# omnirevolve/omnirevolve-image-processor

Hardware: AMD Instinct MI355X
Metric: Mpx/s end-to-end (color->order) (higher is better)
Workload: dtype u8/i32 raster + f32/f64 geometry; 1 GPU; 4096x4096 BGR image, 8 colour layers, stages 02->12 (k-means fit, masks, edges, contours, scale, sort, intra dedup, cross dedup, plot order), default A4 canvas 8400x11880; parallelism=one GPU, one pipeline per colour layer, ops_last_step_rank0=4261, exchange=none

## Files before the change

### omnirevolve-image-processor_amd/csrc/vec_common.h

```cpp
#pragma once
#include "orip_ctx.h"
#include "vec_serial.h"
#include "vsrc.h"
#include <algorithm>
#include <chrono>
#include <string>

template <class T> int vscan_excl(orip_ctx* c, const T* in, T* out, size_t n);
template <class K, class V> int vsort_pairs(orip_ctx* c, const K* kin, K* kout, const V* vin, V* vout, size_t n, int begin_bit, int end_bit, bool desc = false);
template <class T>
static inline int vread(orip_ctx* c, T* host, const T* dev, size_t n = 1) {
    HIPC(c, hipMemcpyAsync(host, dev, n * sizeof(T), hipMemcpyDeviceToHost, LN(c).stream));
    HIPC(c, hipStreamSynchronize(LN(c).stream));
    return 0;
}
struct PhaseTimer {
    orip_ctx* c; const bool on; std::string log; std::chrono::steady_clock::time_point prev;
    PhaseTimer(orip_ctx* ctx, const char* env) : c(ctx), on(getenv(env) != nullptr), prev(std::chrono::steady_clock::now()) {}
    double lap() {
        if (on) hipStreamSynchronize(LN(c).stream);
        const auto t = std::chrono::steady_clock::now(); const double ms = std::chrono::duration<double, std::milli>(t - prev).count(); prev = t;
        return ms;
    }
    void tick(const char* name) { if (on) { char b[64]; snprintf(b, sizeof b, " %s %.2f", name, lap()); log += b; } }
};

struct PolyFeat {
    int32_t x0, y0, x1, y1;
    int32_t sx, sy, ex, ey;
    int64_t n;
    float per;
    double arc;
    uint8_t closed;
};

#define ORIP_LONG_POLY 192
#define ORIP_LONG_CUM 128
static_assert(ORIP_LONG_POLY >= ORIP_LONG_CUM, "every polyline whose perimeter is summed from stored segment lengths must have had them stored");
static inline ESrc esrc_of(const DPolys& P) { return ESrc{P.off.as<int64_t>(), reinterpret_cast<const int2*>(P.pts.p)}; }
int vsrc_of(orip_ctx* c, const DPolys& P, VSrc& out);
#define ORIP_WITH_SRC(c, P, SRC, BODY)                                                         \
    do {                                                                                       \
        if (is_coded(P)) { VSrc SRC; ORIP_TRY(vsrc_of(c, P, SRC)); BODY }                      \
        else { const ESrc SRC = esrc_of(P); BODY }                                             \
    } while (0)
__device__ __forceinline__ int64_t last_le(const int64_t* off, int64_t n, int64_t v) {
    int64_t lo = 0, hi = n - 1;
    while (lo < hi) { const int64_t mid = (lo + hi + 1) >> 1; if (off[mid] <= v) lo = mid; else hi = mid - 1; }
    return lo;
}
__device__ __forceinline__ int64_t ub_u32(const unsigned* a, int64_t n, unsigned v) {
    int64_t lo = 0, hi = n;
    while (lo < hi) { int64_t mid = (lo + hi) >> 1; if (a[mid] <= v) lo = mid + 1; else hi = mid; }
    return lo;
}
template <class Cur> struct CurPt {
    Cur& c;
    __device__ __forceinline__ vs::IPt operator()(int64_t i) const { const int2 p = c.at(i); return vs::IPt{p.x, p.y}; }
};
enum : int {
    VF_PER = 1,
    VF_PER_HYPOT = 2,
    VF_ARC_CLOSED = 4,
    VF_ARC_OPEN = 8,
    VF_OPEN_VIEW = 16,
    VF_PER_REV = 32,
    VF_LEAVES_DONE = 64,
};
int vfeatures(orip_ctx* c, const DPolys& P, int what, PolyFeat* feat);
void vfeatures_short(orip_ctx* c, const VSrc& src, int64_t n, int what, PolyFeat* feat, float* per_rev);
int vlen_order(orip_ctx* c, const int64_t* off, int64_t n, unsigned* kin, unsigned* kout, unsigned* vin, unsigned* order);
int vfeatures_long_seg(orip_ctx* c, const VSrc& src, int64_t n, int64_t total, PolyFeat* feat, const unsigned* order, float* per_rev, const float* seg);
void vwalk_arcs(orip_ctx* c, const VSrc& src, int64_t n, PolyFeat* feat);

struct GatherDesc { int64_t begin; int64_t len; int32_t rev; int32_t src; };
int vgather(orip_ctx* c, const GatherDesc* d, int64_t n, const int32_t* src, DPolys& dst, int64_t known_total = -1);
int vgather_views(orip_ctx* c, const GatherDesc* d, int64_t n, const DPolys& src, DPolys& dst, int64_t known_total = -1);
int vgather_list(orip_ctx* c, const GatherDesc* d, int64_t n, const DPolys& src, DPolys& dst, int64_t known_total = -1);

#define ORIP_RUN_TILE 4096u
struct SlotPtsI2 { const int2* p; __device__ __forceinline__ int2 at(unsigned s) const { return p[s]; } };
struct SlotPtsF64 {
    const double* x; const double* y;
    __device__ __forceinline__ int2 at(unsigned s) const { return make_int2((int)x[s], (int)y[s]); }
};
template <class Pts> int orip_runs_to_polys(orip_ctx* c, Pts pts, const uint8_t* sflag, unsigned n_slots, DPolys& dst);

int vreorder(orip_ctx* c, DPolys& src, DPolys& dst, int kind, const orip_params08* prefetch08 = nullptr);
```

### omnirevolve-image-processor_amd/csrc/vector08a.hip

```cpp
#include "vec08.h"
#include <rocprim/rocprim.hpp>
#include <type_traits>
#include <vector>

namespace {

template <class Src>
__global__ __launch_bounds__(128) void k_split_small08(Src src, int64_t n_polys, orip_params08 P, const PolyFeat* __restrict__ feat,
                                                        unsigned* __restrict__ is_tap, unsigned* __restrict__ is_keep, int2* __restrict__ tap_xy, GatherDesc* __restrict__ kd) {
    int64_t i = (int64_t)blockIdx.x * blockDim.x + threadIdx.x;
    if (i > n_polys) return;
    if (i == n_polys) { is_tap[i] = 0; is_keep[i] = 0; return; }
    const int64_t n = src.len(i);
    unsigned tap = 0, keep = 0;
    GatherDesc g; g.begin = src.off[i]; g.len = n; g.rev = 0; g.src = (int32_t)i;
    if (n >= 2) {
        const int32_t x0 = feat[i].x0, x1 = feat[i].x1, y0 = feat[i].y0, y1 = feat[i].y1;
        double d = (double)max(x1 - x0, y1 - y0);
        if (d <= P.tap_diam && d <= P.tap_max_dim && n <= (int64_t)P.tap_max_v) {
            double per; float cx, cy, r;
            if constexpr (std::is_same<Src, ESrc>::value) {
                const int32_t* p = reinterpret_cast<const int32_t*>(src.pts + src.off[i]);
                per = (double)vs::pairwise_seglen_sum<0>(p, n);
                if (per <= P.tap_max_per) vs::min_enclosing_circle(p, n, cx, cy, r);
            } else {
                auto cu = src.cur(i);
                LocalPts<decltype(cu), 64> lp; lp.load(cu, (int)n);
                per = (double)vs::pairwise_seglen_sum<0>(lp.xy, n);
                if (per <= P.tap_max_per) vs::min_enclosing_circle(lp.xy, n, cx, cy, r);
            }
            if (per <= P.tap_max_per) { tap = 1; tap_xy[i] = make_int2((int)vs::round_half_even((double)cx), (int)vs::round_half_even((double)cy)); }
        }
        if (!tap && !(d < P.min_keep)) {
            keep = 1;
            if (feat[i].closed) g.len = n - 1;
        }
    }
    is_tap[i] = tap; is_keep[i] = keep; kd[i] = g;
}
template <class T>
__global__ __launch_bounds__(256) void k_compact(const unsigned* __restrict__ flag, const unsigned* __restrict__ scan, int64_t n, const T* __restrict__ in, T* __restrict__ out) {
    int64_t i = (int64_t)blockIdx.x * 256 + threadIdx.x;
    if (i < n && flag[i]) out[scan[i]] = in[i];
}

struct RsInfo { int64_t n_eff; double total; unsigned m; unsigned pass; };
__device__ __forceinline__ void rs_finish(RsInfo& r, float acc, int64_t n, double step) {
    r.total = (double)acc;
    if (r.total <= step) { r.pass = 1; r.m = (unsigned)n; }
    else r.m = (unsigned)ceil(r.total / step);
    if (r.m < 2) r.m = 0;
}
template <class Src>
__global__ __launch_bounds__(128) void k_cumlen(Src src, int64_t n_polys, double step, float* __restrict__ cum, RsInfo* __restrict__ info) {
    int64_t i = (int64_t)blockIdx.x * blockDim.x + threadIdx.x;
    if (i >= n_polys) return;
    auto cu = src.cur(i); int64_t n = src.len(i);
    float* s = cum + src.off[i];
    RsInfo r; r.n_eff = n; r.total = 0; r.m = 0; r.pass = 0;
    const int2 pf = cu.at(0);
    auto same_as_first = [&](int64_t k) { const int2 q = cu.at(k); return q.x == pf.x && q.y == pf.y; };
    if (n >= 2 && same_as_first(n - 1)) n -= 1;
    r.n_eff = n;
    if (n >= 2) {
        if (n > 2 && same_as_first(n - 1)) n -= 1;
        r.n_eff = n;
        if (n <= ORIP_LONG_CUM) {
            const CurPt<decltype(cu)> pt{cu};
            float acc = 0.f; s[0] = 0.f;
            for (int64_t k = 0; k + 1 < n; k++) { float sl = vs::seg_len_f32_p(pt, k); acc = (k == 0) ? sl : acc + sl; s[k + 1] = acc; }
            rs_finish(r, acc, n, step);
        }
    }
    info[i] = r;
}

__device__ __forceinline__ unsigned wave_incl_scan_u32(unsigned v) {
#define ORIP_DPP_ADD(ctrl, rowmask) v += (unsigned)__builtin_amdgcn_update_dpp(0, (int)v, ctrl, rowmask, 0xf, false);
    ORIP_DPP_ADD(0x111, 0xf) ORIP_DPP_ADD(0x112, 0xf) ORIP_DPP_ADD(0x114, 0xf) ORIP_DPP_ADD(0x118, 0xf)
    ORIP_DPP_ADD(0x142, 0xa) ORIP_DPP_ADD(0x143, 0xc)
#undef ORIP_DPP_ADD
    return v;
}
__device__ __forceinline__ unsigned wave_incl_scan_max_u32(unsigned v) {
#define ORIP_DPP_MAX(ctrl, rowmask) { const unsigned t_ = (unsigned)__builtin_amdgcn_update_dpp(0, (int)v, ctrl, rowmask, 0xf, false); v = t_ > v ? t_ : v; }
    ORIP_DPP_MAX(0x111, 0xf) ORIP_DPP_MAX(0x112, 0xf) ORIP_DPP_MAX(0x114, 0xf) ORIP_DPP_MAX(0x118, 0xf)
    ORIP_DPP_MAX(0x142, 0xa) ORIP_DPP_MAX(0x143, 0xc)
#undef ORIP_DPP_MAX
    return v;
}
__device__ __forceinline__ float cum_window(float dval, int lane, unsigned& E, unsigned& M) {
    const unsigned b = __float_as_uint(dval);
    const unsigned Ed = b >> 23, Md = Ed ? ((b & 0x7fffffu) | 0x800000u) : 0u;
    unsigned out = 0u; int first = 0;
    for (;;) {
        const int sh = (int)E - (int)Ed;
        const unsigned sc = (unsigned)(sh < 0 ? 0 : (sh > 31 ? 31 : sh));
        const unsigned rem = Md & ((1u << sc) - 1u), half = (1u << sc) >> 1;
        const bool live = lane >= first;
        const bool ev = live && (sh < 0 || (sc > 0u && rem == half));
        const unsigned r = (live && sh >= 0) ? (Md >> sc) + ((sc > 0u && rem > half) ? 1u : 0u) : 0u;
        const unsigned S = wave_incl_scan_u32(r);
        const unsigned long long em = __ballot(ev || (live && M + S >= 0x1000000u));
        const int f = em ? __builtin_ctzll(em) : 64;
        if (live && lane < f) out = (E << 23) | ((M + S) & 0x7fffffu);
        if (f == 64) { M += (unsigned)__builtin_amdgcn_readlane((int)S, 63); break; }
        const unsigned Mp = M + (f > first ? (unsigned)__builtin_amdgcn_readlane((int)S, f - 1) : 0u);
        const float pprev = __uint_as_float((E << 23) | (Mp & 0x7fffffu));
        const float pnew = __fadd_rn(pprev, __uint_as_float((unsigned)__builtin_amdgcn_readlane((int)b, f)));
        const unsigned nb = __float_as_uint(pnew);
        if (lane == f) out = nb;
        E = nb >> 23; M = E ? ((nb & 0x7fffffu) | 0x800000u) : 0u;
        first = f + 1;
        if (first == 64) break;
    }
    return __uint_as_float(out);
}
__device__ __forceinline__ float cum_state_value(unsigned E, unsigned M) { return __uint_as_float((E << 23) | (M & 0x7fffffu)); }
template <class Src>
__global__ __launch_bounds__(128) void k_cumlen2(Src src, const PolyFeat* __restrict__ feat07, int64_t n_polys, double step, float* __restrict__ cum, int64_t rev_off, RsInfo* __restrict__ info) {
    const int64_t gi = (int64_t)blockIdx.x * blockDim.x + threadIdx.x;
    if (gi >= 2 * n_polys) return;
    const int64_t i = gi < n_polys ? gi : gi - n_polys; const int dir0 = gi < n_polys ? 0 : 1;
    auto cu = src.cur(i); const int64_t nfull = src.len(i);
    const bool closed = feat07[i].closed != 0;
    for (int dir = dir0; dir <= dir0; dir++) {
        int64_t n = (dir == 0 && closed && nfull > 0) ? nfull - 1 : nfull;
        float* s = cum + (dir ? rev_off : 0) + src.off[i];
        auto P = [&](int64_t k) { return dir ? cu.at(nfull - 1 - k) : cu.at(k); };
        RsInfo r; r.n_eff = n; r.total = 0; r.m = 0; r.pass = 0;
        if (dir == 1 && closed) { r.n_eff = 0; info[n_polys + i] = r; continue; }
        const int2 pf = P(0);
        auto same_as_first = [&](int64_t k) { const int2 q = P(k); return q.x == pf.x && q.y == pf.y; };
        if (n >= 2 && same_as_first(n - 1)) n -= 1;
        r.n_eff = n;
        if (n >= 2) {
            if (n > 2 && same_as_first(n - 1)) n -= 1;
            r.n_eff = n;
            if (n <= ORIP_LONG_CUM) {
                float acc = 0.f; s[0] = 0.f;
                int2 a = P(0);
                for (int64_t k = 0; k + 1 < n; k++) {
                    const int2 b = P(k + 1);
                    float dx = (float)b.x - (float)a.x, dy = (float)b.y - (float)a.y; float qx = dx * dx, qy = dy * dy; const float sl = sqrtf(qx + qy);
                    acc = (k == 0) ? sl : acc + sl; s[k + 1] = acc; a = b;
                }
                rs_finish(r, acc, n, step);
            }
        }
        info[dir ? n_polys + i : i] = r;
    }
}
__device__ __forceinline__ int2 lane_succ(const int2 v, const int2 last, int lane) {
    int2 r;
    r.x = __builtin_amdgcn_update_dpp(0, v.x, 0x130 , 0xf, 0xf, true);
    r.y = __builtin_amdgcn_update_dpp(0, v.y, 0x130, 0xf, 0xf, true);
    if (lane == 63) r = last;
    return r;
}
template <class Src>
__device__ __forceinline__ void cumlen_long_wave(const Src& src, int64_t n_polys, double step, float* __restrict__ cum, int64_t rev_off, RsInfo* __restrict__ info,
                                                 const unsigned* __restrict__ ord, const bool rev, const float* __restrict__ seg, int64_t slot, int64_t n_slots, const int lane) {
    for (int64_t rr = slot; rr < n_polys; rr += n_slots) {
        const int64_t i = ord[rr];
        RsInfo r = info[rev ? n_polys + i : i];
        if (r.n_eff <= ORIP_LONG_CUM) continue;
        auto cu = src.cur(i); const int64_t nfull = src.len(i);
        float* s = cum + (rev ? rev_off : 0) + src.off[i];
        const int64_t ns = r.n_eff - 1;
        const float* sg = seg ? seg + src.off[i] : nullptr;
        const bool from_seg = sg != nullptr;
        float acc = 0.f; unsigned cE = 0u, cM = 0u;
        if (lane == 0) s[0] = 0.f;
        auto P = [&](int64_t k) { return cu.at(rev ? nfull - 1 - k : k); };
        auto request = [&](int64_t base, int2 (&p)[5], float (&fl)[4]) {
            if (from_seg) {
#pragma unroll
                for (int w = 0; w < 4; w++) { const int64_t k = base + 64 * w + lane; fl[w] = k < ns ? sg[rev ? nfull - 2 - k : k] : 0.f; }
            } else {
#pragma unroll
                for (int w = 0; w < 4; w++) { const int64_t k = base + 64 * w + lane; p[w] = k <= ns ? P(k) : make_int2(0, 0); }
                p[4] = base + 256 <= ns ? P(base + 256) : make_int2(0, 0);
            }
        };
        auto lengths = [&](int64_t base, const int2 (&p)[5], const float (&fl)[4], float (&sl)[4]) {
            if (from_seg) {
#pragma unroll
                for (int w = 0; w < 4; w++) sl[w] = fl[w];
                return;
            }
#pragma unroll
            for (int w = 0; w < 4; w++) {
                const int64_t k = base + 64 * w + lane;
                const int2 nx0 = w < 3 ? make_int2(__builtin_amdgcn_readlane(p[w + 1].x, 0), __builtin_amdgcn_readlane(p[w + 1].y, 0)) : p[4];
                const int2 b2 = lane_succ(p[w], nx0, lane);
                float dx = (float)b2.x - (float)p[w].x, dy = (float)b2.y - (float)p[w].y; float qx = dx * dx, qy = dy * dy;
                const float L = sqrtf(qx + qy);
                sl[w] = k < ns ? L : 0.f;
            }
        };
        int2 rp[5]; float rf[4] = {0.f, 0.f, 0.f, 0.f}; float cur[4];
        request(0, rp, rf); lengths(0, rp, rf, cur);
        for (int64_t base = 0; base < ns; base += 256) {
            request(base + 256, rp, rf);
#pragma unroll
            for (int w = 0; w < 4; w++) {
                const int64_t k = base + 64 * w + lane;
                const float pv = cum_window(cur[w], lane, cE, cM); acc = cum_state_value(cE, cM);
                if (k < ns) s[k + 1] = pv;
            }
            lengths(base + 256, rp, rf, cur);
        }
        if (lane == 0) { rs_finish(r, acc, r.n_eff, step); info[rev ? n_polys + i : i] = r; }
    }
}
template <class Src>
__global__ __launch_bounds__(64) void k_cumlen_long2(Src src, int64_t n_polys, double step, float* __restrict__ cum, int64_t rev_off, RsInfo* __restrict__ info, const unsigned* __restrict__ ord,
                                                     int dir0, const float* __restrict__ seg) {
    cumlen_long_wave<Src>(src, n_polys, step, cum, rev_off, info, ord, ((blockIdx.y + (unsigned)dir0) & 1u) != 0, seg, blockIdx.x, gridDim.x, threadIdx.x);
}
template <class Src>
__global__ __launch_bounds__(256) void k_seglen(Src src, int64_t n_polys, int64_t total, float* __restrict__ seg, PolyFeat* __restrict__ bb) {
    const int lane = threadIdx.x & 63;
    const int64_t base = ((int64_t)blockIdx.x * 4 + (threadIdx.x >> 6)) * (63 * 64);
    if (base >= total) return;
    int64_t g = base + lane;
    int64_t i = 0;
    { const int64_t gg = g < total ? g : total - 1; int64_t hi = n_polys - 1;
      while (i < hi) { const int64_t mid = (i + hi + 1) >> 1; if (src.off[mid] <= gg) i = mid; else hi = mid - 1; } }
    int64_t o0 = src.off[i], o1 = src.off[i + 1];
    auto cu = src.cur(i);
    bool is_long = o1 - o0 > ORIP_LONG_CUM;
    int64_t vn = is_long ? bb[i].n : 0; if (vn <= ORIP_LONG_POLY) vn = 0;
    int bx0 = 0x7fffffff, bx1 = -0x7fffffff, by0 = 0x7fffffff, by1 = -0x7fffffff; bool has = false;
    for (int t = 0; t < 64 && base + 63 * t < total; t++, g += 63) {
        const bool valid = g < total;
        if (valid && g >= o1) {
            if (has) { atomicMin(&bb[i].x0, bx0); atomicMax(&bb[i].x1, bx1); atomicMin(&bb[i].y0, by0); atomicMax(&bb[i].y1, by1); }
            bx0 = by0 = 0x7fffffff; bx1 = by1 = -0x7fffffff; has = false;
            do { i++; o0 = o1; o1 = src.off[i + 1]; } while (g >= o1);
            cu = src.cur(i); is_long = o1 - o0 > ORIP_LONG_CUM;
            vn = is_long ? bb[i].n : 0; if (vn <= ORIP_LONG_POLY) vn = 0;
        }
// ... 881 lines not shown
```

### omnirevolve-image-processor_amd/csrc/vector_greedy.hip

```cpp
#include "vec_common.h"

namespace {
struct NNEnds { int32_t sx, sy, ex, ey; uint8_t closed; };
__device__ __forceinline__ float nn_d2(int32_t ax, int32_t ay, int32_t bx, int32_t by) {
    float dx = __fsub_rn((float)ax, (float)bx), dy = __fsub_rn((float)ay, (float)by);
    return __fadd_rn(__fmul_rn(dx, dx), __fmul_rn(dy, dy));
}
enum : int { NN_BEYOND_I16 = 1, NN_BEYOND_15BIT = 2 };
#define ORIP_NN_GATE(sel, skip_if, need_any) const int fl_ = (sel)[1]; if ((fl_ & (skip_if)) != 0 || ((need_any) != 0 && (fl_ & (need_any)) == 0)) return; const int seed = (sel)[0];
__device__ __forceinline__ bool nn_direction(bool cl, float ds, float de, bool& flip) { flip = cl ? false : !(ds <= de); return cl || flip; }
struct NNCand { int32_t sx, sy, ex, ey; bool cl, used; };
struct NNStoreGlobal {
    static constexpr int THREADS = 0;
    const NNEnds* ends; uint8_t* used; int rule07;
    __device__ __forceinline__ NNStoreGlobal(const NNEnds* e, int, int r07, uint8_t* u) : ends(e), used(u), rule07(r07) {}
    __device__ __forceinline__ void init(int i, int seed) { used[i] = (i == seed); }
    __device__ __forceinline__ NNCand load(int i) const {
        NNCand q; q.used = used[i] != 0; if (q.used) return q;
        const NNEnds e = ends[i]; q.sx = e.sx; q.sy = e.sy; q.ex = e.ex; q.ey = e.ey; q.cl = rule07 && e.closed;
        return q;
    }
    __device__ __forceinline__ void mark_used(int i) { used[i] = 1; }
};
struct NNStoreLds {
// ... 288 lines not shown
        "v_cmp_gt_u32_e64 s[92:93], s74, v42\n\t"
        "v_cmp_gt_u32_e64 s[96:97], s74, v43\n\t"
        "s_waitcnt lgkmcnt(0)\n\t"
        ORIP_NN_FETCH("v66", "v70", "v65", "68", "69")
        ORIP_NN_FETCH("v76", "v71", "v73", "74", "75")
        "s_waitcnt lgkmcnt(0)\n\t"
        ORIP_NN_KEY("v70", "v67", "68", "69", "s[92:93]")
        ORIP_NN_KEY("v71", "v77", "74", "75", "s[96:97]")
        ORIP_NN_MERGE("66", "67", "68", "69", "v65")
        ORIP_NN_MERGE("76", "77", "74", "75", "v73")
        "s_add_i32 s98, s98, 128\n\t"
        "s_cmp_lt_u32 s98, s74\n\t"
        "s_cbranch_scc1 L_pair%=\n\t"
        "L_best%=:\n\t"
        "v_mov_b32 v47, v59\n\t"
        "v_and_b32 v54, 0x7fff7fff, v52\n\t"
        "v_and_b32 v64, 1, v58\n\t"
        "v_min_u32_dpp v47, v47, v47 row_shr:1 row_mask:0xf bank_mask:0xf\n\t"
        "v_cmp_ne_u32 vcc, 0, v64\n\t"
        "v_cmp_gt_i32_e64 s[90:91], 0, v52\n\t"
        "v_min_u32_dpp v47, v47, v47 row_shr:2 row_mask:0xf bank_mask:0xf\n\t"
        "v_cndmask_b32 v62, v53, v54, vcc\n\t"
        "v_or_b32 v60, 0x8000, v52\n\t"
        "v_min_u32_dpp v47, v47, v47 row_shr:4 row_mask:0xf bank_mask:0xf\n\t"
        "v_cndmask_b32_e64 v62, v62, v54, s[90:91]\n\t"
        "s_nop 0\n\t"
        "v_min_u32_dpp v47, v47, v47 row_shr:8 row_mask:0xf bank_mask:0xf\n\t"
        "s_nop 1\n\t"
        "v_min_u32_dpp v47, v47, v47 row_bcast:15 row_mask:0xa bank_mask:0xf\n\t"
        "s_nop 1\n\t"
        "v_min_u32_dpp v47, v47, v47 row_bcast:31 row_mask:0xc bank_mask:0xf\n\t"
        "s_nop 1\n\t"
        "v_readlane_b32 s77, v47, 63\n\t"
        "s_cmp_eq_u32 s77, -1\n\t"
        "s_cbranch_scc1 L_fb5%=\n\t"
        "v_cvt_u32_f32 v48, s77\n\t"
        "v_add_u32 v48, 1, v48\n\t"
        "v_cmp_ge_u32 vcc, s59, v48\n\t"
        "s_and_b64 s[94:95], vcc, exec\n\t"
        "s_cbranch_scc0 L_gap%=\n\t"
        "L_gapok%=:\n\t"
        "v_cmp_eq_u32_e64 s[82:83], s77, v59\n\t"
        "s_bcnt1_i32_b64 s79, s[82:83]\n\t"
        "s_cmp_eq_u32 s79, 1\n\t"
        "s_cbranch_scc1 L_win%=\n\t"
        "v_cndmask_b32_e64 v47, -1, v58, s[82:83]\n\t"
        ORIP_NN_MIN6
        "v_readlane_b32 s79, v47, 63\n\t"
        "s_nop 1\n\t"
        "v_cmp_eq_u32_e64 s[94:95], s79, v58\n\t"
        "s_and_b64 s[82:83], s[82:83], s[94:95]\n\t"
        "L_win%=:\n\t"
        "s_ff1_i32_b64 s84, s[82:83]\n\t"
        "v_readlane_b32 s85, v58, s84\n\t"
        "v_readlane_b32 s86, v62, s84\n\t"
        "s_mov_b64 s[90:91], exec\n\t"
        "s_mov_b64 exec, s[82:83]\n\t"
        "ds_write_b32 v51, v60\n\t"
        "s_mov_b64 exec, s[90:91]\n\t"
        "v_writelane_b32 %[ringv], s85, m0\n\t"
        "s_lshr_b32 s79, s85, 1\n\t"
        "s_cmp_eq_u32 s58, 2\n\t"
        "s_cbranch_scc1 L_upd2%=\n\t"
        "v_lshrrev_b32 v50, 1, v49\n\t"
        "v_or_b32 v55, 0x8000, v52\n\t"
        "v_cmp_eq_u32 vcc, s79, v50\n\t"
        "v_cndmask_b32 v52, v52, v55, vcc\n\t"
        "s_branch L_next%=\n\t"
        "L_upd2%=:\n\t"
        "v_lshrrev_b32 v50, 1, v66\n\t"
        "v_or_b32 v55, 0x8000, v68\n\t"
        "v_cmp_eq_u32 vcc, s79, v50\n\t"
        "v_cndmask_b32 v68, v68, v55, vcc\n\t"
        "v_lshrrev_b32 v50, 1, v76\n\t"
        "v_or_b32 v55, 0x8000, v74\n\t"
        "v_cmp_eq_u32 vcc, s79, v50\n\t"
        "v_cndmask_b32 v74, v74, v55, vcc\n\t"
        "L_next%=:\n\t"
        "s_and_b32 %[cx], s86, 0xffff\n\t"
        "s_lshr_b32 %[cy], s86, 16\n\t"
        "v_cvt_f32_i32 v40, %[cx]\n\t"
        "v_cvt_f32_i32 v41, %[cy]\n\t"
        "s_add_i32 %[step], %[step], 1\n\t"
        "s_add_i32 m0, m0, 1\n\t"
        "s_cmp_eq_u32 m0, 64\n\t"
        "s_cbranch_scc1 L_flush%=\n\t"
        "s_cmp_ge_u32 %[step], %[n]\n\t"
        "s_cbranch_scc1 L_done%=\n\t"
        "s_branch L_step%=\n\t"
        "L_gap%=:\n\t"
        "s_and_b32 s79, %[cx], s88\n\t"
        "s_sub_i32 s80, s87, s79\n\t"
        "s_add_i32 s79, s79, 1\n\t"
        "s_min_i32 s79, s79, s80\n\t"
        "s_and_b32 s80, %[cy], s88\n\t"
        "s_sub_i32 s78, s87, s80\n\t"
        "s_add_i32 s80, s80, 1\n\t"
        "s_min_i32 s80, s80, s78\n\t"
        "s_min_i32 s79, s79, s80\n\t"
        "s_add_i32 s79, s79, s87\n\t"
        "s_mul_i32 s78, s79, s79\n\t"
        "s_lshr_b32 s80, s78, 18\n\t"
        "s_sub_i32 s78, s78, s80\n\t"
        "s_add_i32 s78, s78, -1\n\t"
        "v_cmp_ge_u32 vcc, s78, v48\n\t"
        "s_and_b64 s[94:95], vcc, exec\n\t"
        "s_cbranch_scc1 L_gapok%=\n\t"
        "s_mov_b32 %[ev], 6\n\t"
        "s_branch L_out%=\n\t"
        "L_hit1%=:\n\t"
        "s_add_i32 %[cnt], %[cnt], 1\n\t"
        "s_branch L_key%=\n\t"
        "L_hit2%=:\n\t"
        "s_add_i32 %[cnt], %[cnt], 0x400\n\t"
        "s_branch L_key2%=\n\t"
        "L_fb3%=:\n\t"
        "s_mov_b32 %[ev], 3\n\t"
        "s_branch L_out%=\n\t"
        "L_fb5%=:\n\t"
        "s_mov_b32 %[ev], 5\n\t"
        "s_branch L_out%=\n\t"
        "L_flush%=:\n\t"
        "s_mov_b32 %[ev], 1\n\t"
        "s_branch L_out%=\n\t"
        "L_done%=:\n\t"
        "s_mov_b32 %[ev], 0\n\t"
        "L_out%=:\n\t"
        "s_waitcnt lgkmcnt(0)\n\t"
        "s_mov_b32 m0, s89\n\t"
        : [ev] "=&s"(ev), [cx] "+s"(s_cx), [cy] "+s"(s_cy), [step] "+s"(s_step), [ringv] "+v"(ringv), [cnt] "+s"(s_cnt)
        : [n] "s"(s_n), [sh] "s"(s_sh), [G] "s"(s_G), [Gm1] "s"(s_Gm1), [cstb] "s"(s_cst), [eidb] "s"(s_eid), [pb] "s"(s_p), [nem1] "s"(s_nem1),
          [rowoff] "v"(rowoff), [isend] "v"(isend), [lane] "v"(lane)
        : "vcc", "scc", "memory",
          "s58", "s59", "s60", "s61", "s62", "s63", "s64", "s65", "s66", "s67", "s68", "s69", "s70", "s71", "s72", "s73", "s74", "s75", "s76", "s77", "s78", "s79", "s80", "s81",
          "s82", "s83", "s84", "s85", "s86", "s87", "s88", "s89", "s90", "s91", "s92", "s93", "s94", "s95", "s96", "s97", "s98",
          "v40", "v41", "v42", "v43", "v44", "v45", "v46", "v47", "v48", "v49", "v50", "v51", "v52", "v53", "v54", "v55", "v56", "v57", "v58", "v59", "v60",
          "v61", "v62", "v63", "v64", "v65", "v66", "v67", "v68", "v69", "v70", "v71", "v72", "v73", "v74", "v75", "v76", "v77");
#undef ORIP_NN_Q
#undef ORIP_NN_FETCH
#undef ORIP_NN_KEY
#undef ORIP_NN_MERGE
#undef ORIP_NN_MIN6
    cx = s_cx; cy = s_cy; step = s_step; dbg_cnt = s_cnt;
    return ev;
}

__global__ __launch_bounds__(64) void k_greedy_nn_fast(const NNEnds* __restrict__ ends, int n, const int* __restrict__ sel, int skip_if, int need_any, int rule07, int G,
                                                        int32_t* __restrict__ order, uint8_t* __restrict__ flips, int no_asm, unsigned long long* __restrict__ dbg) {
    ORIP_NN_GATE(sel, skip_if, need_any)
    extern __shared__ __align__(16) unsigned char smem[];
    uint2* P = reinterpret_cast<uint2*>(smem);
    unsigned* cst = reinterpret_cast<unsigned*>(P + n);
    uint16_t* Eid = reinterpret_cast<uint16_t*>(cst + (G * G + 2));
    const int lane = threadIdx.x;
#define NNU(x) __builtin_amdgcn_readfirstlane((int)(x))
    int mnx = 0x7fffffff, mny = 0x7fffffff, mxx = -0x7fffffff, mxy = -0x7fffffff;
    for (int i = lane; i < n; i += 64) {
        NNEnds e = ends[i];
        mnx = min(mnx, min(e.sx, e.ex)); mxx = max(mxx, max(e.sx, e.ex)); mny = min(mny, min(e.sy, e.ey)); mxy = max(mxy, max(e.sy, e.ey));
    }
    for (int o = 32; o > 0; o >>= 1) { mnx = min(mnx, __shfl_xor(mnx, o, 64)); mny = min(mny, __shfl_xor(mny, o, 64)); mxx = max(mxx, __shfl_xor(mxx, o, 64)); mxy = max(mxy, __shfl_xor(mxy, o, 64)); }
    const int ox = mnx, oy = mny;
    for (int i = lane; i < n; i += 64) {
        NNEnds e = ends[i];
        P[i] = make_uint2((unsigned)((e.sx - ox) | (i == seed ? 0x8000 : 0)) | ((unsigned)((e.sy - oy) | ((rule07 && e.closed) ? 0x8000 : 0)) << 16),
                          (unsigned)(e.ex - ox) | ((unsigned)(e.ey - oy) << 16));
    }
    unsigned* cnt = cst + 1;
    for (int i = lane; i <= G * G + 1; i += 64) cst[i] = 0;
    __syncthreads();
    int sh = 0; while (((max(mxx - mnx, mxy - mny)) >> sh) >= G) sh++;
    sh = NNU(sh);
    for (int i = lane; i < n; i += 64) {
        const uint2 e = P[i];
        atomicAdd(&cnt[(((e.x >> 16) & 0x7fff) >> sh) * G + ((e.x & 0x7fff) >> sh)], 1u);
        if (!(e.x & 0x80000000u)) atomicAdd(&cnt[((e.y >> 16) >> sh) * G + ((e.y & 0xffff) >> sh)], 1u);
    }
    __syncthreads();
    {
        const int per = (G * G + 63) / 64, c0 = lane * per, c1 = min(G * G, c0 + per);
        unsigned sm = 0;
        for (int cc = c0; cc < c1; cc++) sm += cnt[cc];
        unsigned inc = sm;
        for (int o = 1; o < 64; o <<= 1) { unsigned t = __shfl_up(inc, o, 64); if (lane >= o) inc += t; }
        unsigned run = inc - sm;
        for (int cc = c0; cc < c1; cc++) { unsigned v = cnt[cc]; cnt[cc] = run; run += v; }
    }
    __syncthreads();
    for (int i = lane; i < n; i += 64) {
        const uint2 e = P[i];
        Eid[atomicAdd(&cnt[(((e.x >> 16) & 0x7fff) >> sh) * G + ((e.x & 0x7fff) >> sh)], 1u)] = (uint16_t)(i << 1);
        if (!(e.x & 0x80000000u)) Eid[atomicAdd(&cnt[((e.y >> 16) >> sh) * G + ((e.y & 0xffff) >> sh)], 1u)] = (uint16_t)((i << 1) | 1);
    }
    __syncthreads();
    const unsigned n_ent = (unsigned)NNU(cst[G * G]);
    int cx, cy;
    { const uint2 e = P[seed]; const bool cl = (e.x & 0x80000000u) != 0; cx = NNU(cl ? (e.x & 0x7fff) : (e.y & 0xffff)); cy = NNU(cl ? ((e.x >> 16) & 0x7fff) : (e.y >> 16)); }
    unsigned ringv = lane == 0 ? (unsigned)(seed << 1) : 0u;
    const int Gm1 = G - 1;
    const bool use_asm = G >= 4 && !no_asm;
    const unsigned lds_p = (unsigned)(uintptr_t)P, lds_cst = (unsigned)(uintptr_t)cst, lds_eid = (unsigned)(uintptr_t)Eid;
    const int rowoff = lane < 6 ? (lane >> 1) : 0, isend = lane < 6 ? (lane & 1) : 0;
    int step = 1, r_first = 1;
    unsigned long long d_fb = 0, d_calls = 0, t_asm = 0, t_gen = 0;
    while (step < n) {
        if (use_asm) {
            const unsigned long long t_0 = dbg ? __builtin_amdgcn_s_memtime() : 0ull;
            int cnt = 0;
            const int ev = nn_asm_steps(cx, cy, step, ringv, n, sh, G, lds_p, lds_cst, lds_eid, n_ent - 1u, rowoff, isend, lane, cnt);
            if (dbg) { t_asm += __builtin_amdgcn_s_memtime() - t_0; d_calls++; if (lane == 0) { if (ev >= 2) dbg[2 + ev]++; dbg[4] += (unsigned)cnt & 0x3ffu; dbg[6] += ((unsigned)cnt >> 10) & 0x3ffu; dbg[9] += (unsigned)cnt >> 20; } }
            if (ev == 1) { order[step - 64 + lane] = (int32_t)(ringv >> 1); flips[step - 64 + lane] = (uint8_t)(ringv & 1u); continue; }
            if (ev == 0) break;
            r_first = 3;
        }
        const unsigned long long t_g0 = dbg ? __builtin_amdgcn_s_memtime() : 0ull;
        d_fb++;
        const int gx = cx >> sh, gy = cy >> sh;
        const float fx = (float)cx, fy = (float)cy;
        unsigned wi = 0, w0 = 0, w1 = 0;
        for (int r = r_first;; r = 2 * r + 1) {
            const int x0 = max(0, gx - r), x1 = min(Gm1, gx + r), y0 = max(0, gy - r), y1 = min(Gm1, gy + r);
            unsigned myk = ~0u, myi = 0x7fffffffu, my0 = 0, my1 = 0;
            auto consider = [&](unsigned q, bool valid) {
                const unsigned id = Eid[q < n_ent ? q : n_ent - 1u]; const unsigned i = id >> 1;
                const uint2 e = P[i];
                const unsigned xy = (id & 1u) ? e.y : (e.x & 0x7fff7fffu);
                const float dx = __fsub_rn((float)(xy & 0xffffu), fx), dy = __fsub_rn((float)(xy >> 16), fy);
                unsigned k = __float_as_uint(__fadd_rn(__fmul_rn(dx, dx), __fmul_rn(dy, dy)));
                k = (valid && !(e.x & 0x8000u)) ? k : ~0u;
                const unsigned long long key = ((unsigned long long)k << 32) | i, mine = ((unsigned long long)myk << 32) | myi;
                const bool better = key < mine;
                myk = better ? k : myk; myi = better ? i : myi; my0 = better ? e.x : my0; my1 = better ? e.y : my1;
            };
            if (y1 - y0 <= 2) {
                const int row = y0 + (lane >> 1);
                const int ci = row * G + ((lane & 1) ? x1 + 1 : x0);
                const unsigned bnd = (lane < 6 && row <= y1) ? cst[ci] : 0u;
                const unsigned lo0 = (unsigned)__builtin_amdgcn_readlane((int)bnd, 0), n0 = (unsigned)__builtin_amdgcn_readlane((int)bnd, 1) - lo0;
                const unsigned lo1 = (unsigned)__builtin_amdgcn_readlane((int)bnd, 2), n1 = (unsigned)__builtin_amdgcn_readlane((int)bnd, 3) - lo1;
                const unsigned lo2 = (unsigned)__builtin_amdgcn_readlane((int)bnd, 4), n2 = (unsigned)__builtin_amdgcn_readlane((int)bnd, 5) - lo2;
                const unsigned n01 = n0 + n1, total = n01 + n2;
                for (unsigned t0 = 0; t0 < total; t0 += 64) {
                    const unsigned t = t0 + lane;
                    unsigned q = lo0 + t;
                    q = t >= n0 ? lo1 + (t - n0) : q;
                    q = t >= n01 ? lo2 + (t - n01) : q;
                    consider(q, t < total);
                }
            } else {
                for (int row = y0; row <= y1; row++) {
                    const unsigned lo = (unsigned)NNU(cst[row * G + x0]), hi = (unsigned)NNU(cst[row * G + x1 + 1]);
                    for (unsigned q0 = lo; q0 < hi; q0 += 64) consider(q0 + lane, q0 + lane < hi);
                }
            }
            unsigned m = myk;
#define ORIP_DPP_MINU(ctrl, rmask) { const unsigned t_ = (unsigned)__builtin_amdgcn_update_dpp((int)0xffffffffu, (int)m, ctrl, rmask, 0xf, false); m = t_ < m ? t_ : m; }
            ORIP_DPP_MINU(0x111, 0xf) ORIP_DPP_MINU(0x112, 0xf) ORIP_DPP_MINU(0x114, 0xf) ORIP_DPP_MINU(0x118, 0xf) ORIP_DPP_MINU(0x142, 0xa) ORIP_DPP_MINU(0x143, 0xc)
#undef ORIP_DPP_MINU
            const unsigned mink = (unsigned)__builtin_amdgcn_readlane((int)m, 63);
            bool final_ = x0 == 0 && y0 == 0 && x1 == Gm1 && y1 == Gm1;
            if (!final_ && mink != ~0u) {
                int gap;
                if (r == 1) {
                    const int cell = 1 << sh, lx = cx & (cell - 1), ly = cy & (cell - 1);
                    gap = cell + min(min(lx + 1, cell - lx), min(ly + 1, cell - ly));
                } else {
                    gap = 0x7fff;
                    if (x0 > 0) gap = min(gap, cx - (x0 << sh) + 1);
                    if (x1 < Gm1) gap = min(gap, ((x1 + 1) << sh) - cx);
                    if (y0 > 0) gap = min(gap, cy - (y0 << sh) + 1);
                    if (y1 < Gm1) gap = min(gap, ((y1 + 1) << sh) - cy);
                }
                const unsigned g2 = (unsigned)(gap * gap);
                const unsigned bfl = (unsigned)NNU((unsigned)__uint_as_float(mink));
                final_ = bfl + 1u <= g2 - (g2 >> 18) - 1u && g2 > 1u;
            }
            if (final_) {
                unsigned long long tie = __ballot(myk == mink);
                if (tie & (tie - 1)) {
                    unsigned ci2 = myk == mink ? myi : 0x7fffffffu;
                    for (int o = 32; o > 0; o >>= 1) { const unsigned t_ = (unsigned)__shfl_xor((int)ci2, o, 64); ci2 = t_ < ci2 ? t_ : ci2; }
                    tie = __ballot(myk == mink && myi == ci2);
                }
                const unsigned sxy = my0 & 0x7fff7fffu;
                const float ds = nn_d2((int)(sxy & 0xffffu), (int)(sxy >> 16), cx, cy), de = nn_d2((int)(my1 & 0xffffu), (int)(my1 >> 16), cx, cy);
                const bool cl = (my0 & 0x80000000u) != 0;
                bool flip;
                const unsigned ncur = nn_direction(cl, ds, de, flip) ? sxy : my1;
                const unsigned pack = (myi << 1) | (flip ? 1u : 0u);
                const int win_lane = __ffsll((long long)tie) - 1;
                wi = (unsigned)__builtin_amdgcn_readlane((int)pack, win_lane);
                w1 = (unsigned)__builtin_amdgcn_readlane((int)ncur, win_lane);
                w0 = (unsigned)__builtin_amdgcn_readlane((int)my0, win_lane);
                break;
            }
        }
        P[wi >> 1].x = w0 | 0x8000u;
        ringv = lane == (step & 63) ? wi : ringv;
        if ((step & 63) == 63) { order[step - 63 + lane] = (int32_t)(ringv >> 1); flips[step - 63 + lane] = (uint8_t)(ringv & 1u); }
        cx = (int)(w1 & 0xffffu); cy = (int)(w1 >> 16);
        step++;
        if (dbg) t_gen += __builtin_amdgcn_s_memtime() - t_g0;
    }
    if (dbg && lane == 0) { dbg[0] = d_fb; dbg[1] = d_calls; dbg[2] = t_asm; dbg[3] = t_gen; }
    { const int done = n & ~63; if (done + lane < n) { order[done + lane] = (int32_t)(ringv >> 1); flips[done + lane] = (uint8_t)(ringv & 1u); } }
#undef NNU
}
}

static int nn_dbg2_report(orip_ctx* c, unsigned long long* dbg, int kind, int64_t n, int G) {
    unsigned long long h[10];
    HIPC(c, hipStreamSynchronize(LN(c).stream)); HIPC(c, hipMemcpy(h, dbg, 80, hipMemcpyDeviceToHost));
    fprintf(stderr, "[nn dbg2] kind %d n %lld G %d: %llu steps by the compiled code (empty %llu, all used %llu, gap %llu; asm steps from cached candidates: "
                    "one per lane %llu, two per lane %llu; with more than 128 candidates %llu), %llu asm entries, cycles asm %llu compiled %llu\n",
            kind, (long long)n, G, h[0], h[5], h[7], h[8], h[4], h[6], h[9], h[1], h[2], h[3]);
    HIPC(c, hipMemsetAsync(dbg, 0, 80, LN(c).stream));
    return 0;
}
int vreorder(orip_ctx* c, DPolys& src, DPolys& dst, int kind, const orip_params08* prefetch08) {
    int64_t n = src.n;
    if (n == 0) { HIPC(c, dst.clear(LN(c).stream)); return 0; }
    if (n > 0x7fffffff) ORIP_FAIL(c, "too many polylines");
    PolyFeat* feat; NNEnds* ends; GatherDesc* desc; int32_t* order; uint8_t *flips, *used;
    { Carve L; L.each(n, feat, ends, desc, order, flips, used); HIPC(c, L.commit(LN(c).vtmp[VTL_FEAT], 256)); }
    const int what = kind == 7 ? VF_ARC_CLOSED : (kind == 8 ? VF_PER : VF_ARC_OPEN);
    if (kind == 7 && is_coded(src) && src.vident && !getenv("ORIP_ARC_POINTS")) {
        VSrc vs_; ORIP_TRY(vsrc_of(c, src, vs_));
        vfeatures_short(c, vs_, n, what, feat, nullptr);
        if (src.total > ORIP_LONG_POLY) { ProfScope ps(c, "k_walk_arcs"); vwalk_arcs(c, vs_, n, feat); }
        HIPC(c, hipGetLastError());
    } else ORIP_TRY(vfeatures(c, src, what, feat));
    ORIP_WITH_SRC(c, src, ps, { hipLaunchKernelGGL(k_ends_from_feat<decltype(ps)>, dim3(cdiv(n, 256)), dim3(256), 0, LN(c).stream, feat, n, kind == 7 ? 1 : 0, ps, ends); });
    LaneFlags* fl = LN(c).flags.as<LaneFlags>(); int* d_seed = fl->nn_seed;
    hipLaunchKernelGGL(k_argmax_feat, dim3(1), dim3(256), 0, LN(c).stream, feat, (int)n, kind == 8 ? 0 : 1, d_seed, ends);
    const size_t lds = (size_t)n * 9 + 16;
    int G = 8; while (G < 128 && (size_t)(G + 8) * (G + 8) <= 4 * (size_t)n && (size_t)n * 12 + (size_t)((G + 8) * (G + 8) + 1) * 4 + 64 <= 158 * 1024) G += 8;
    const size_t lds_grid = (size_t)n * 12 + (size_t)(G * G + 1) * 4 + 64;
    static std::once_flag attr_once;
    static std::atomic<int> attr_err{0};
    std::call_once(attr_once, [] {
        orip_max_lds(k_greedy_nn<NNStoreLds>, 150 * 1024, attr_err);
        orip_max_lds(k_greedy_nn_fast, 158 * 1024, attr_err);
    });
    if (attr_err.load()) ORIP_FAIL(c, "hipFuncSetAttribute(greedy kernels) failed: %s", hipGetErrorString((hipError_t)attr_err.load()));
    if (prefetch08) HIPC(c, hipEventRecord(LN(c).ev2, LN(c).stream));
    const bool grid_ok = n >= 64 && n <= 16000 && lds_grid <= 158 * 1024 && !getenv("ORIP_NN_NOGRID");
    const bool lds_ok = n <= 16000;
    const int r07 = kind == 7 ? 1 : 0;
    {
        ProfScope ps(c, "k_greedy_nn");
        if (grid_ok) {
            unsigned long long* dbg2 = getenv("ORIP_NN_DBG2") ? fl->nn_dbg2 : nullptr;
            if (dbg2) HIPC(c, hipMemsetAsync(dbg2, 0, 80, LN(c).stream));
            hipLaunchKernelGGL(k_greedy_nn_fast, dim3(1), dim3(64), lds_grid + 4, LN(c).stream, ends, (int)n, d_seed, NN_BEYOND_I16 | NN_BEYOND_15BIT, 0, r07, G, order, flips, getenv("ORIP_NN_NOASM") ? 1 : 0, dbg2);
            if (dbg2) ORIP_TRY(nn_dbg2_report(c, dbg2, kind, n, G));
        }
        if (lds_ok && !grid_ok) hipLaunchKernelGGL(k_greedy_nn<NNStoreLds>, dim3(1), dim3(1024), lds, LN(c).stream, ends, (int)n, d_seed, NN_BEYOND_I16, 0, r07, (uint8_t*)nullptr, order, flips);
        const int need = grid_ok ? (NN_BEYOND_I16 | NN_BEYOND_15BIT) : (lds_ok ? NN_BEYOND_I16 : 0);
        hipLaunchKernelGGL(k_greedy_nn<NNStoreGlobal>, dim3(1), dim3(lds_ok ? 256 : 1024), 0, LN(c).stream, ends, (int)n, d_seed, 0, need, r07, used, order, flips);
    }
    if (prefetch08) ORIP_TRY(orip_prefetch08(c, *prefetch08, src, feat));
    hipLaunchKernelGGL(k_desc_from_order, dim3(cdiv(n, 256)), dim3(256), 0, LN(c).stream, src.off.as<int64_t>(), order, flips, n, 0, feat, desc);
    HIPC(c, hipGetLastError());
    return vgather_list(c, desc, n, src, dst, src.total);
}
```

Before: 283.1 Mpx/s.

## Flatten multi-row grid candidate scan in greedy NN with wave scan compaction

In the grid-based greedy nearest-neighbour kernel, wide search windows previously looped row by row, issuing 64-lane batches per row even when rows held few candidates. The new path reads up to 64 rows' cell ranges at once and prefix-scans their counts across the wave. An LDS table plus a max-scan then maps each lane to its candidate, so 128 candidates are processed per iteration with two loads in flight per lane. This adds LDS, atomic stores and a fence per batch, and it also adds debug counters.

```diff
diff --git a/omnirevolve-image-processor_amd/csrc/vec_common.h b/omnirevolve-image-processor_amd/csrc/vec_common.h
--- a/omnirevolve-image-processor_amd/csrc/vec_common.h
+++ b/omnirevolve-image-processor_amd/csrc/vec_common.h
@@ -54,6 +54,20 @@
     while (lo < hi) { int64_t mid = (lo + hi) >> 1; if (a[mid] <= v) lo = mid + 1; else hi = mid; }
     return lo;
 }
+__device__ __forceinline__ unsigned wave_incl_scan_u32(unsigned v) {
+#define ORIP_DPP_ADD(ctrl, rowmask) v += (unsigned)__builtin_amdgcn_update_dpp(0, (int)v, ctrl, rowmask, 0xf, false);
+    ORIP_DPP_ADD(0x111, 0xf) ORIP_DPP_ADD(0x112, 0xf) ORIP_DPP_ADD(0x114, 0xf) ORIP_DPP_ADD(0x118, 0xf)
+    ORIP_DPP_ADD(0x142, 0xa) ORIP_DPP_ADD(0x143, 0xc)
+#undef ORIP_DPP_ADD
+    return v;
+}
+__device__ __forceinline__ unsigned wave_incl_scan_max_u32(unsigned v) {
+#define ORIP_DPP_MAX(ctrl, rowmask) { const unsigned t_ = (unsigned)__builtin_amdgcn_update_dpp(0, (int)v, ctrl, rowmask, 0xf, false); v = t_ > v ? t_ : v; }
+    ORIP_DPP_MAX(0x111, 0xf) ORIP_DPP_MAX(0x112, 0xf) ORIP_DPP_MAX(0x114, 0xf) ORIP_DPP_MAX(0x118, 0xf)
+    ORIP_DPP_MAX(0x142, 0xa) ORIP_DPP_MAX(0x143, 0xc)
+#undef ORIP_DPP_MAX
+    return v;
+}
 template <class Cur> struct CurPt {
     Cur& c;
     __device__ __forceinline__ vs::IPt operator()(int64_t i) const { const int2 p = c.at(i); return vs::IPt{p.x, p.y}; }
diff --git a/omnirevolve-image-processor_amd/csrc/vector08a.hip b/omnirevolve-image-processor_amd/csrc/vector08a.hip
--- a/omnirevolve-image-processor_amd/csrc/vector08a.hip
+++ b/omnirevolve-image-processor_amd/csrc/vector08a.hip
@@ -75,20 +75,6 @@
     info[i] = r;
 }
 
-__device__ __forceinline__ unsigned wave_incl_scan_u32(unsigned v) {
-#define ORIP_DPP_ADD(ctrl, rowmask) v += (unsigned)__builtin_amdgcn_update_dpp(0, (int)v, ctrl, rowmask, 0xf, false);
-    ORIP_DPP_ADD(0x111, 0xf) ORIP_DPP_ADD(0x112, 0xf) ORIP_DPP_ADD(0x114, 0xf) ORIP_DPP_ADD(0x118, 0xf)
-    ORIP_DPP_ADD(0x142, 0xa) ORIP_DPP_ADD(0x143, 0xc)
-#undef ORIP_DPP_ADD
-    return v;
-}
-__device__ __forceinline__ unsigned wave_incl_scan_max_u32(unsigned v) {
-#define ORIP_DPP_MAX(ctrl, rowmask) { const unsigned t_ = (unsigned)__builtin_amdgcn_update_dpp(0, (int)v, ctrl, rowmask, 0xf, false); v = t_ > v ? t_ : v; }
-    ORIP_DPP_MAX(0x111, 0xf) ORIP_DPP_MAX(0x112, 0xf) ORIP_DPP_MAX(0x114, 0xf) ORIP_DPP_MAX(0x118, 0xf)
-    ORIP_DPP_MAX(0x142, 0xa) ORIP_DPP_MAX(0x143, 0xc)
-#undef ORIP_DPP_MAX
-    return v;
-}
 __device__ __forceinline__ float cum_window(float dval, int lane, unsigned& E, unsigned& M) {
     const unsigned b = __float_as_uint(dval);
     const unsigned Ed = b >> 23, Md = Ed ? ((b & 0x7fffffu) | 0x800000u) : 0u;
diff --git a/omnirevolve-image-processor_amd/csrc/vector_greedy.hip b/omnirevolve-image-processor_amd/csrc/vector_greedy.hip
--- a/omnirevolve-image-processor_amd/csrc/vector_greedy.hip
+++ b/omnirevolve-image-processor_amd/csrc/vector_greedy.hip
@@ -464,6 +464,8 @@
     uint2* P = reinterpret_cast<uint2*>(smem);
     unsigned* cst = reinterpret_cast<unsigned*>(P + n);
     uint16_t* Eid = reinterpret_cast<uint16_t*>(cst + (G * G + 2));
+    unsigned* wtab = reinterpret_cast<unsigned*>(Eid + 2 * n);
+    const unsigned long long t_k0 = dbg ? __builtin_amdgcn_s_memtime() : 0ull;
     const int lane = threadIdx.x;
 #define NNU(x) __builtin_amdgcn_readfirstlane((int)(x))
     int mnx = 0x7fffffff, mny = 0x7fffffff, mxx = -0x7fffffff, mxy = -0x7fffffff;
@@ -515,6 +517,8 @@
     const int rowoff = lane < 6 ? (lane >> 1) : 0, isend = lane < 6 ? (lane & 1) : 0;
     int step = 1, r_first = 1;
     unsigned long long d_fb = 0, d_calls = 0, t_asm = 0, t_gen = 0;
+    unsigned d_rounds = 0, d_cand = 0;
+    if (dbg && lane == 0) dbg[9] = (__builtin_amdgcn_s_memtime() - t_k0) << 32;
     while (step < n) {
         if (use_asm) {
             const unsigned long long t_0 = dbg ? __builtin_amdgcn_s_memtime() : 0ull;
@@ -533,17 +537,24 @@
         for (int r = r_first;; r = 2 * r + 1) {
             const int x0 = max(0, gx - r), x1 = min(Gm1, gx + r), y0 = max(0, gy - r), y1 = min(Gm1, gy + r);
             unsigned myk = ~0u, myi = 0x7fffffffu, my0 = 0, my1 = 0;
-            auto consider = [&](unsigned q, bool valid) {
-                const unsigned id = Eid[q < n_ent ? q : n_ent - 1u]; const unsigned i = id >> 1;
-                const uint2 e = P[i];
-                const unsigned xy = (id & 1u) ? e.y : (e.x & 0x7fff7fffu);
+            d_rounds++;
+            struct Cand { unsigned k, i; uint2 e; };
+            auto fetch = [&](unsigned q, bool valid) {
+                const unsigned id = Eid[q < n_ent ? q : n_ent - 1u]; Cand c; c.i = id >> 1;
+                c.e = P[c.i];
+                const unsigned xy = (id & 1u) ? c.e.y : (c.e.x & 0x7fff7fffu);
                 const float dx = __fsub_rn((float)(xy & 0xffffu), fx), dy = __fsub_rn((float)(xy >> 16), fy);
-                unsigned k = __float_as_uint(__fadd_rn(__fmul_rn(dx, dx), __fmul_rn(dy, dy)));
-                k = (valid && !(e.x & 0x8000u)) ? k : ~0u;
-                const unsigned long long key = ((unsigned long long)k << 32) | i, mine = ((unsigned long long)myk << 32) | myi;
+                const unsigned k = __float_as_uint(__fadd_rn(__fmul_rn(dx, dx), __fmul_rn(dy, dy)));
+                c.k = (valid && !(c.e.x & 0x8000u)) ? k : ~0u;
+                return c;
+            };
+            auto merge = [&](const Cand& c) {
+                const unsigned long long key = ((unsigned long long)c.k << 32) | c.i, mine = ((unsigned long long)myk << 32) | myi;
                 const bool better = key < mine;
-                myk = better ? k : myk; myi = better ? i : myi; my0 = better ? e.x : my0; my1 = better ? e.y : my1;
+                myk = better ? c.k : myk; myi = better ? c.i : myi; my0 = better ? c.e.x : my0; my1 = better ? c.e.y : my1;
             };
+            auto consider = [&](unsigned q, bool valid) { merge(fetch(q, valid)); };
+            auto consider2 = [&](unsigned qa, bool va, unsigned qb, bool vb) { const Cand a = fetch(qa, va), b = fetch(qb, vb); merge(a); merge(b); };
             if (y1 - y0 <= 2) {
                 const int row = y0 + (lane >> 1);
                 const int ci = row * G + ((lane & 1) ? x1 + 1 : x0);
@@ -552,6 +563,7 @@
                 const unsigned lo1 = (unsigned)__builtin_amdgcn_readlane((int)bnd, 2), n1 = (unsigned)__builtin_amdgcn_readlane((int)bnd, 3) - lo1;
                 const unsigned lo2 = (unsigned)__builtin_amdgcn_readlane((int)bnd, 4), n2 = (unsigned)__builtin_amdgcn_readlane((int)bnd, 5) - lo2;
                 const unsigned n01 = n0 + n1, total = n01 + n2;
+                if (dbg) d_cand += total;
                 for (unsigned t0 = 0; t0 < total; t0 += 64) {
                     const unsigned t = t0 + lane;
                     unsigned q = lo0 + t;
@@ -560,9 +572,25 @@
                     consider(q, t < total);
                 }
             } else {
-                for (int row = y0; row <= y1; row++) {
-                    const unsigned lo = (unsigned)NNU(cst[row * G + x0]), hi = (unsigned)NNU(cst[row * G + x1 + 1]);
-                    for (unsigned q0 = lo; q0 < hi; q0 += 64) consider(q0 + lane, q0 + lane < hi);
+                for (int yc = y0; yc <= y1; yc += 64) {
+                    const int row = min(yc + lane, y1);
+                    const unsigned lo = cst[row * G + x0], hi = cst[row * G + x1 + 1];
+                    const unsigned cn = yc + lane <= y1 ? hi - lo : 0u;
+                    const unsigned incl = wave_incl_scan_u32(cn), excl = incl - cn;
+                    const unsigned total = (unsigned)__builtin_amdgcn_readlane((int)incl, 63);
+                    const unsigned word = (excl << 16) | lo;
+                    if (dbg) d_cand += total;
+                    for (unsigned t0 = 0; t0 < total; t0 += 128) {
+                        __hip_atomic_store(&wtab[lane], 0u, __ATOMIC_RELAXED, __HIP_MEMORY_SCOPE_WAVEFRONT);
+                        __hip_atomic_store(&wtab[64 + lane], 0u, __ATOMIC_RELAXED, __HIP_MEMORY_SCOPE_WAVEFRONT);
+                        __hip_atomic_store(&wtab[(cn != 0u && excl < t0 + 128u && incl > t0) ? max(excl, t0) - t0 : 128u], word, __ATOMIC_RELAXED, __HIP_MEMORY_SCOPE_WAVEFRONT);
+                        __builtin_amdgcn_fence(__ATOMIC_ACQ_REL, "wavefront");
+                        const unsigned wa = wave_incl_scan_max_u32(__hip_atomic_load(&wtab[lane], __ATOMIC_RELAXED, __HIP_MEMORY_SCOPE_WAVEFRONT));
+                        unsigned wb = wave_incl_scan_max_u32(__hip_atomic_load(&wtab[64 + lane], __ATOMIC_RELAXED, __HIP_MEMORY_SCOPE_WAVEFRONT));
+                        wb = max(wb, (unsigned)__builtin_amdgcn_readlane((int)wa, 63));
+                        const unsigned ta = t0 + lane, tb = ta + 64u;
+                        consider2((wa & 0xffffu) + (ta - (wa >> 16)), ta < total, (wb & 0xffffu) + (tb - (wb >> 16)), tb < total);
+                    }
                 }
             }
             unsigned m = myk;
@@ -614,7 +642,7 @@
         step++;
         if (dbg) t_gen += __builtin_amdgcn_s_memtime() - t_g0;
     }
-    if (dbg && lane == 0) { dbg[0] = d_fb; dbg[1] = d_calls; dbg[2] = t_asm; dbg[3] = t_gen; }
+    if (dbg && lane == 0) { dbg[0] = d_fb | ((unsigned long long)d_rounds << 32); dbg[1] = d_calls | ((unsigned long long)d_cand << 32); dbg[2] = t_asm; dbg[3] = t_gen; }
     { const int done = n & ~63; if (done + lane < n) { order[done + lane] = (int32_t)(ringv >> 1); flips[done + lane] = (uint8_t)(ringv & 1u); } }
 #undef NNU
 }
@@ -623,9 +651,11 @@
 static int nn_dbg2_report(orip_ctx* c, unsigned long long* dbg, int kind, int64_t n, int G) {
     unsigned long long h[10];
     HIPC(c, hipStreamSynchronize(LN(c).stream)); HIPC(c, hipMemcpy(h, dbg, 80, hipMemcpyDeviceToHost));
+    const unsigned long long lo32 = 0xffffffffull;
     fprintf(stderr, "[nn dbg2] kind %d n %lld G %d: %llu steps by the compiled code (empty %llu, all used %llu, gap %llu; asm steps from cached candidates: "
-                    "one per lane %llu, two per lane %llu; with more than 128 candidates %llu), %llu asm entries, cycles asm %llu compiled %llu\n",
-            kind, (long long)n, G, h[0], h[5], h[7], h[8], h[4], h[6], h[9], h[1], h[2], h[3]);
+                    "one per lane %llu, two per lane %llu; with more than 128 candidates %llu), %llu asm entries, cycles asm %llu compiled %llu; "
+                    "compiled rounds %llu with %llu candidates, prologue cycles %llu\n",
+            kind, (long long)n, G, h[0] & lo32, h[5], h[7], h[8], h[4], h[6], h[9] & lo32, h[1] & lo32, h[2], h[3], h[0] >> 32, h[1] >> 32, h[9] >> 32);
     HIPC(c, hipMemsetAsync(dbg, 0, 80, LN(c).stream));
     return 0;
 }
@@ -648,11 +678,12 @@
     const size_t lds = (size_t)n * 9 + 16;
     int G = 8; while (G < 128 && (size_t)(G + 8) * (G + 8) <= 4 * (size_t)n && (size_t)n * 12 + (size_t)((G + 8) * (G + 8) + 1) * 4 + 64 <= 158 * 1024) G += 8;
     const size_t lds_grid = (size_t)n * 12 + (size_t)(G * G + 1) * 4 + 64;
+    constexpr size_t NN_WTAB_BYTES = 129 * 4;
     static std::once_flag attr_once;
     static std::atomic<int> attr_err{0};
     std::call_once(attr_once, [] {
         orip_max_lds(k_greedy_nn<NNStoreLds>, 150 * 1024, attr_err);
-        orip_max_lds(k_greedy_nn_fast, 158 * 1024, attr_err);
+        orip_max_lds(k_greedy_nn_fast, 158 * 1024 + 4 + (int)NN_WTAB_BYTES, attr_err);
     });
     if (attr_err.load()) ORIP_FAIL(c, "hipFuncSetAttribute(greedy kernels) failed: %s", hipGetErrorString((hipError_t)attr_err.load()));
     if (prefetch08) HIPC(c, hipEventRecord(LN(c).ev2, LN(c).stream));
@@ -664,7 +695,7 @@
         if (grid_ok) {
             unsigned long long* dbg2 = getenv("ORIP_NN_DBG2") ? fl->nn_dbg2 : nullptr;
             if (dbg2) HIPC(c, hipMemsetAsync(dbg2, 0, 80, LN(c).stream));
-            hipLaunchKernelGGL(k_greedy_nn_fast, dim3(1), dim3(64), lds_grid + 4, LN(c).stream, ends, (int)n, d_seed, NN_BEYOND_I16 | NN_BEYOND_15BIT, 0, r07, G, order, flips, getenv("ORIP_NN_NOASM") ? 1 : 0, dbg2);
+            hipLaunchKernelGGL(k_greedy_nn_fast, dim3(1), dim3(64), lds_grid + 4 + NN_WTAB_BYTES, LN(c).stream, ends, (int)n, d_seed, NN_BEYOND_I16 | NN_BEYOND_15BIT, 0, r07, G, order, flips, getenv("ORIP_NN_NOASM") ? 1 : 0, dbg2);
             if (dbg2) ORIP_TRY(nn_dbg2_report(c, dbg2, kind, n, G));
         }
         if (lds_ok && !grid_ok) hipLaunchKernelGGL(k_greedy_nn<NNStoreLds>, dim3(1), dim3(1024), lds, LN(c).stream, ends, (int)n, d_seed, NN_BEYOND_I16, 0, r07, (uint8_t*)nullptr, order, flips);
```

New measurement: 287.9 Mpx/s, median of 6. +1.7%, better.
